# k-flouris/cmf

Measured on AMD Instinct MI355X. Metric: log-density evals/sec (JtJ-cholesky path), MNIST D=784 d=64 bs=512, higher is better.
Workload: dtype f32 (3x3 tangent convs as bf16x3 split MFMA, fp32 accumulate); 1 GPU; C3: MNIST-shaped (1,28,28) uint8-range + U[0,1) noise, non-square flow d=64, cholesky J^T J log-det + g_ij off-diagonal L1 + reconstruction, eval/no_grad; per_gpu_batch=512, global_batch=512, D=784, latent_dimension=64, parallelism=dp1

## Files before the change

cmf_amd/csrc/conv_block_head.hip:

```cpp
#include <stdint.h>

#include "common.h"

namespace {

typedef __bf16 bf16x8 __attribute__((ext_vector_type(8)));
typedef __bf16 bf16x2 __attribute__((ext_vector_type(2)));
typedef float f32x2 __attribute__((ext_vector_type(2)));
typedef unsigned u32x4 __attribute__((ext_vector_type(4)));

constexpr int HID = 64, KJ = HID * 9, NT = 512, ROWS = 16, ND = 25, HALO = 8, XB = 4;
constexpr int SLICE = HID * 16;
static_assert(2 * KJ > 2 * NT && 2 * KJ <= 3 * NT && (2 * KJ - 2 * NT) % 64 == 0, "phase B: two units per thread, a third for whole waves");
constexpr int W1_FRAGS = 9 * 4 * 2 * 2 * 64;

__device__ __forceinline__ unsigned pack_hi(float a, float b, float& ra, float& rb) {
  bf16x2 h = __builtin_convertvector(f32x2{a, b}, bf16x2);
  const unsigned bits = __builtin_bit_cast(unsigned, h);
  ra = a - __builtin_bit_cast(float, bits << 16);
  rb = b - __builtin_bit_cast(float, bits & 0xffff0000u);
  return bits;
}
__device__ __forceinline__ unsigned pack_lo(float a, float b) {
  bf16x2 h = __builtin_convertvector(f32x2{a, b}, bf16x2);
  return __builtin_bit_cast(unsigned, h);
}

__global__ void pack_block_weight_kernel(const float* __restrict__ w, u32x4* __restrict__ out) {
  const int idx = blockIdx.x * 256 + threadIdx.x;
  if (idx >= W1_FRAGS) return;
  const int l = idx & 63, hl = (idx >> 6) & 1, ks = (idx >> 7) & 1, ct = (idx >> 8) & 3, t1 = idx >> 10;
  const int c = 16 * ct + (l & 15), ci0 = 32 * ks + 8 * (l >> 4);
  unsigned r[4];
#pragma unroll
  for (int jj = 0; jj < 4; ++jj) {
    const float v0 = w[((ci0 + 2 * jj) * HID + c) * 9 + t1], v1 = w[((ci0 + 2 * jj + 1) * HID + c) * 9 + t1];
    float ra, rb;
    const unsigned h = pack_hi(v0, v1, ra, rb);
    r[jj] = hl ? pack_lo(ra, rb) : h;
  }
  out[idx] = u32x4{r[0], r[1], r[2], r[3]};
}

struct Tile {
  int row0, s0, xb, Ws, H, W, live;
  __device__ __forceinline__ bool slot(int p, int& row, int& col, int& po) const {
    const int s = s0 + (p & 1);
    row = row0 + (p >> 1);
    col = live ? 2 * s + ((row + live - 1) & 1) : s;
    po = row * Ws + s;
    return row < H && s < Ws;
  }
};

__device__ __forceinline__ void load_w1(u32x4 (&b)[2][2], const u32x4* __restrict__ wp, int ct, int lane, int t1) {
#pragma unroll
  for (int ks = 0; ks < 2; ++ks)
#pragma unroll
    for (int hl = 0; hl < 2; ++hl) b[ks][hl] = wp[(((t1 * 4 + ct) * 2 + ks) * 2 + hl) * 64 + lane];
}

template <int HALF, int CP>
__device__ __forceinline__ void build_half(const u32x4* __restrict__ wp, const u32x4* As, float* Ks, const float* Gs,
                                           const unsigned long long* ha, const int* ctr, int ct, int lane) {
  constexpr int D0 = HALF ? 12 : 0, NDH = HALF ? 13 : 12;
  const f32x4 zero = {0.f, 0.f, 0.f, 0.f};
  f32x4 acc[NDH];
  u32x4 af[9][2][2], bw[2][2][2];
#pragma unroll
  for (int i = 0; i < NDH; ++i) acc[i] = zero;
  load_w1(bw[0], wp, ct, lane, 0);
#pragma unroll
  for (int t2 = 0; t2 < 9; ++t2)
#pragma unroll
    for (int ks = 0; ks < 2; ++ks)
#pragma unroll
      for (int hl = 0; hl < 2; ++hl) af[t2][ks][hl] = As[((t2 * 2 + ks) * 2 + hl) * 64 + lane];
#pragma unroll
  for (int t1 = 0; t1 < 9; ++t1) {
    if (t1 < 8) load_w1(bw[(t1 + 1) & 1], wp, ct, lane, t1 + 1);
#pragma unroll
    for (int t2 = 0; t2 < 9; ++t2) {
      const int d = (t1 / 3 + t2 / 3) * 5 + t1 % 3 + t2 % 3;
      if (d >= D0 && d < D0 + NDH) {
#pragma unroll
        for (int ks = 0; ks < 2; ++ks) {
          const bf16x8 ah = __builtin_bit_cast(bf16x8, af[t2][ks][0]), al = __builtin_bit_cast(bf16x8, af[t2][ks][1]);
          const bf16x8 bh = __builtin_bit_cast(bf16x8, bw[t1 & 1][ks][0]), bl = __builtin_bit_cast(bf16x8, bw[t1 & 1][ks][1]);
          acc[d - D0] = __builtin_amdgcn_mfma_f32_16x16x32_bf16(al, bh, acc[d - D0], 0, 0, 0);
          acc[d - D0] = __builtin_amdgcn_mfma_f32_16x16x32_bf16(ah, bl, acc[d - D0], 0, 0, 0);
          acc[d - D0] = __builtin_amdgcn_mfma_f32_16x16x32_bf16(ah, bh, acc[d - D0], 0, 0, 0);
        }
      }
    }
  }
  const int c = 16 * ct + (lane & 15);
#pragma unroll
  for (int dl = 0; dl < NDH; ++dl) {
    const int d = D0 + dl;
#pragma unroll
    for (int i = 0; i < 4; ++i) {
      const int row = 4 * (lane >> 4) + i, p = row / CP, o = row % CP;
      const int at = ctr[p];
      const bool on = at >= 0 && ((ha[at + (d / 5 - 2) * HALO + d % 5 - 2] >> c) & 1);
      float v = on ? acc[dl][i] : 0.f;
      if (d == 12) v = Gs[c * ROWS + row] + v;
      Ks[((p * ND + d) * HID + c) * CP + o] = v;
    }
  }
}

template <int R, int CP>
__device__ __forceinline__ void phase_b(const float* __restrict__ w2, const float* Gs, const unsigned long long* um, u32x4* As, int tid) {
  int q[R], rh[R];
  float acc[R][8];
#pragma unroll
  for (int r = 0; r < R; ++r) {
    const int u = tid + r * NT;
    rh[r] = u >= KJ, q[r] = u - rh[r] * KJ;
#pragma unroll
    for (int i = 0; i < 8; ++i) acc[r][i] = 0.f;
  }
#pragma unroll 8
  for (int c = 0; c < HID; ++c) {
    float w[R];
#pragma unroll
    for (int r = 0; r < R; ++r) w[r] = w2[c * KJ + q[r]];
#pragma unroll
    for (int r = 0; r < R; ++r) {
      const f32x4 g0 = *reinterpret_cast<const f32x4*>(&Gs[c * ROWS + rh[r] * 8]), g1 = *reinterpret_cast<const f32x4*>(&Gs[c * ROWS + rh[r] * 8 + 4]);
#pragma unroll
      for (int k = 0; k < 4; ++k) {
        acc[r][k] = fmaf(g0[k], w[r], acc[r][k]);
        acc[r][4 + k] = fmaf(g1[k], w[r], acc[r][4 + k]);
      }
    }
  }
  unsigned short* A16 = reinterpret_cast<unsigned short*>(As);
#pragma unroll
  for (int r = 0; r < R; ++r) {
    const int ci = q[r] / 9, tap = q[r] - ci * 9, ks = ci >> 5, kq = (ci >> 3) & 3, j = ci & 7;
#pragma unroll
    for (int i = 0; i < 8; ++i) {
      const int row = rh[r] * 8 + i, p = row / CP;
      const float e = ((um[p * 9 + tap] >> ci) & 1) ? acc[r][i] : 0.f;
      float ra, rb;
      const unsigned h = pack_hi(e, 0.f, ra, rb);
      const unsigned l = pack_lo(ra, 0.f);
      const int at = ((tap * 2 + ks) * 2 * 64 + kq * 16 + row) * 8 + j;
      A16[at] = (unsigned short)(h & 0xffffu);
      A16[at + 64 * 8] = (unsigned short)(l & 0xffffu);
    }
  }
}

template <int CP>
__global__ __launch_bounds__(NT, 2) void conv_block_head_kernel(cmf_conv_tangent_args a, int tiles_x, int tiles_per_sample, int ntiles) {
  constexpr int P = ROWS / CP, TR = P / 2 > 0 ? P / 2 : 1, PU = P / 2;
  static_assert(P >= 2, "two output columns per tile");
  __shared__ __attribute__((aligned(16))) float Ks[ROWS * ND * HID];
  __shared__ __attribute__((aligned(16))) u32x4 As[9 * 2 * 2 * 64];
  __shared__ __attribute__((aligned(16))) float Gs[HID * ROWS];
  __shared__ unsigned long long um[P * 9];
  __shared__ unsigned long long ha[HALO * HALO];
  __shared__ unsigned long long hl[HALO * HALO];
  __shared__ unsigned long long alv[P];
  __shared__ int ctr[P];

  const int per = (ntiles + 7) >> 3;
  const int item = (int)(blockIdx.x & 7) * per + (int)(blockIdx.x >> 3);
  if (item >= ntiles) return;
  const int b = item / tiles_per_sample, tl = item - b * tiles_per_sample, ty = tl / tiles_x, tx = tl - ty * tiles_x;
  const int tid = threadIdx.x, lane = tid & 63, wv = __builtin_amdgcn_readfirstlane(tid >> 6);
  const int H = a.H, W = a.W, cout = a.head_cout;
  Tile T;
  T.H = H, T.W = W, T.live = a.live, T.Ws = a.live ? W >> 1 : W, T.row0 = ty * TR, T.s0 = 2 * tx, T.xb = a.live ? 4 * tx : 2 * tx;
  const int y0 = T.row0 - 2, x0 = T.xb - 2;

  if (tid < P * 9) {
    const int p = tid / 9, tap = tid - p * 9;
    int row, col, po;
    unsigned long long m = 0;
    if (T.slot(p, row, col, po)) {
      const int r = row + tap / 3 - 1, c = col + tap % 3 - 1;
      if (r >= 0 && r < H && c >= 0 && c < W)
        m = *reinterpret_cast<const unsigned long long*>(reinterpret_cast<const unsigned char*>(a.block_m1) + (long long)b * a.block_m1_np +
                                                         (long long)(r * W + c) * (HID / 8));
    }
    um[tid] = m;
  } else if (tid >= 256 && tid < 256 + HALO * HALO) {
    const int q = tid - 256, r = y0 + (q >> 3), c = x0 + (q & 7);
    unsigned long long m = 0;
    if (r >= 0 && r < H && c >= 0 && c < W)
      m = *reinterpret_cast<const unsigned long long*>(reinterpret_cast<const unsigned char*>(a.f) + (long long)b * a.f_np +
                                                       (long long)(r * W + c) * (HID / 8));
    ha[q] = m;
    hl[q] = m;
  }
  for (int p = wv; p < P; p += NT / 64) {
    int row, col, po;
    const bool ok = T.slot(p, row, col, po);
    bool on = false;
    if (ok) on = a.head_a[(long long)b * a.head_a_np + (long long)lane * a.head_a_c + (long long)(row * W + col) * a.head_a_px] > 0.f;
    const unsigned long long bal = __ballot(on);
    if (lane == 0) {
      alv[p] = bal;
      ctr[p] = ok ? (row - y0) * HALO + (col - x0) : -1;
    }
#pragma unroll
    for (int o = 0; o < CP; ++o) Gs[(lane * P + p) * CP + o] = (on && o < cout) ? a.head_w[o * HID + lane] : 0.f;
  }
  __syncthreads();
  if (tid < P) {
    int row, col, po;
    if (T.slot(tid, row, col, po)) hl[ctr[tid]] |= alv[tid];
  }

  if (wv < (2 * KJ - 2 * NT) / 64)
    phase_b<3, CP>(a.w, Gs, um, As, tid);
  else
    phase_b<2, CP>(a.w, Gs, um, As, tid);
  __syncthreads();

  {
    const u32x4* wp = reinterpret_cast<const u32x4*>(a.block_w1);
    if (wv < 4)
      build_half<0, CP>(wp, As, Ks, Gs, ha, ctr, wv & 3, lane);
    else
      build_half<1, CP>(wp, As, Ks, Gs, ha, ctr, wv & 3, lane);
  }
  __syncthreads();

  const int nsl = a.nc >> 4, cl = lane >> 2;
  const f32x4 zero = {0.f, 0.f, 0.f, 0.f};
  for (int unit = wv; unit < nsl * 2; unit += NT / 64) {
    const int sl = unit >> 1, ph = unit & 1;
    int prow[PU], pcol[PU], ppo[PU];
    bool pok[PU];
    int ylo = H, yhi = -1, xlo = W, xhi = -1;
#pragma unroll
    for (int k = 0; k < PU; ++k) {
      pok[k] = T.slot(ph * PU + k, prow[k], pcol[k], ppo[k]);
      if (pok[k]) {
        ylo = min(ylo, prow[k] - 2), yhi = max(yhi, prow[k] + 2);
        xlo = min(xlo, pcol[k] - 2), xhi = max(xhi, pcol[k] + 2);
      }
    }
    if (yhi < 0) continue;
    ylo = max(ylo, 0), yhi = min(yhi, H - 1), xlo = max(xlo, 0), xhi = min(xhi, W - 1);
    const float* hb = a.x + (long long)b * a.x_np + sl * SLICE + lane * 4;
    f32x4 acc[PU][CP];
#pragma unroll
    for (int k = 0; k < PU; ++k)
#pragma unroll
      for (int o = 0; o < CP; ++o) acc[k][o] = zero;

    for (int y = ylo; y <= yhi; ++y) {
#pragma unroll 1
      for (int xs = xlo; xs <= xhi; xs += XB) {
        f32x4 v[XB][4];
#pragma unroll
        for (int xi = 0; xi < XB; ++xi) {
#pragma unroll
          for (int ch = 0; ch < 4; ++ch) v[xi][ch] = zero;
          const int x = xs + xi;
          if (x <= xhi) {
            const unsigned long long m = hl[(y - y0) * HALO + (x - x0)];
            const float* src = hb + (long long)(y * W + x) * a.x_px;
#pragma unroll
            for (int ch = 0; ch < 4; ++ch)
              if ((m >> (ch * 16 + cl)) & 1) v[xi][ch] = *reinterpret_cast<const f32x4*>(src + ch * 256);
          }
        }
#pragma unroll
        for (int xi = 0; xi < XB; ++xi) {
          const int x = xs + xi;
#pragma unroll
          for (int k = 0; k < PU; ++k) {
            const int dy = y - prow[k] + 2, dx = x - pcol[k] + 2;
            if (x <= xhi && pok[k] && dy >= 0 && dy < 5 && dx >= 0 && dx < 5) {
              const float* coef = &Ks[(((ph * PU + k) * ND + dy * 5 + dx) * HID + cl) * CP];
#pragma unroll
              for (int ch = 0; ch < 4; ++ch) {
                const float* e4 = static_cast<const float*>(__builtin_assume_aligned(coef + ch * 16 * CP, CP < 4 ? 8 : 16));
#pragma unroll
                for (int o = 0; o < CP; ++o) {
                  const float e = e4[o];
#pragma unroll
                  for (int q = 0; q < 4; ++q) acc[k][o][q] = fmaf(e, v[xi][ch][q], acc[k][o][q]);
                }
              }
            }
          }
        }
      }
    }

    constexpr int N = 4 * CP;
#pragma unroll
    for (int k = 0; k < PU; ++k) {
      float val[N];
#pragma unroll
      for (int o = 0; o < CP; ++o)
#pragma unroll
        for (int q = 0; q < 4; ++q) val[4 * o + q] = acc[k][o][q];
#pragma unroll
      for (int s = 0; s < 4; ++s) {
        const int off = 32 >> s, n = N >> s;
        if (n >= 2) {
          const bool hi = lane & off;
#pragma unroll
          for (int i = 0; i < n / 2; ++i) {
            const float mine = hi ? val[n / 2 + i] : val[i], send = hi ? val[i] : val[n / 2 + i];
            val[i] = mine + __shfl_xor(send, off, 64);
          }
        } else {
          val[0] += __shfl_xor(val[0], off, 64);
        }
      }
      if (pok[k]) {
        float* yb = a.head_y + (long long)b * a.head_y_np + (long long)ppo[k] * a.head_y_px + sl * 16 + (lane & 3) * 4;
        constexpr int KEEP = N >= 16 ? N / 16 : 1;
#pragma unroll
        for (int i = 0; i < KEEP; ++i) {
          const int idx = ((cl * N) >> 4) + i, o = idx >> 2;
          if (o < cout && (N >= 16 || !(lane & 4))) yb[(long long)o * a.head_y_co + (idx & 3)] = val[i];
        }
      }
    }
  }
}

template <int CP>
int launch(const cmf_conv_tangent_args& a, hipStream_t s) {
  constexpr int P = ROWS / CP, TR = P / 2;
  const int Ws = a.live ? a.W / 2 : a.W;
  const long long tiles_x = (Ws + 1) / 2, tiles = tiles_x * ((a.H + TR - 1) / TR), ntiles = tiles * a.np;
  if (ntiles > 0x7ffffff0LL) return CMF_ERANGE;
  const int grid = 8 * (int)((ntiles + 7) / 8);
  hipLaunchKernelGGL(conv_block_head_kernel<CP>, dim3(grid), dim3(NT), 0, s, a, (int)tiles_x, (int)tiles, (int)ntiles);
  CMF_LAUNCH_CHECK();
  return 0;
}

}

extern "C" int cmf_pack_block_weight(const float* w, void* out, long long* out_bytes, void* stream) {
  if (!out) {
    if (!out_bytes) return CMF_EINVAL;
    *out_bytes = (long long)W1_FRAGS * 16;
    return 0;
  }
  if (!w || (uintptr_t)out % 16 || (uintptr_t)w % 4) return CMF_EINVAL;
  hipLaunchKernelGGL(pack_block_weight_kernel, dim3((W1_FRAGS + 255) / 256), dim3(256), 0, (hipStream_t)stream, w, (u32x4*)out);
  CMF_LAUNCH_CHECK();
  return 0;
}

int cmf_conv_block_head(const cmf_conv_tangent_args& a, hipStream_t s) {
  if (!a.x || !a.w || !a.f || !a.block_w1 || !a.block_m1 || !a.head_w || !a.head_a || !a.head_y) return CMF_EINVAL;
  if (a.r && a.r != a.x) return CMF_EINVAL;
  if (a.fmode != CMF_F_RELU_BITS || a.taps != 9 || a.cin != HID || a.cout != HID) return CMF_EINVAL;
  if (a.head_cout < 1 || a.head_cout > 8 || a.np <= 0 || a.H <= 0 || a.W <= 0 || a.nc <= 0 || a.nc % 16) return CMF_EINVAL;
  if (a.bias || a.fo || a.ymask || a.mask_out || a.seed || a.live < 0 || a.live > 2 || (a.live && a.W % 2)) return CMF_EINVAL;
  if (!((a.W % 14 == 0 && a.H % 2 == 0) || (a.W % 8 == 0 && a.H % 4 == 0))) return CMF_EINVAL;
  const long long HW = (long long)a.H * a.W;
  if (HW > (1 << 24)) return CMF_ERANGE;
  if (a.x_ci != 16 || a.x_sl != SLICE) return CMF_EINVAL;
  if ((a.x_np | a.x_px | a.head_y_np | a.head_y_co | a.head_y_px) % 4) return CMF_EINVAL;
  if (a.x_px < (long long)HID * a.nc || a.head_y_px < a.nc) return CMF_EINVAL;
  if ((uintptr_t)a.x % 16 || (uintptr_t)a.head_y % 16 || (uintptr_t)a.w % 4 || (uintptr_t)a.head_w % 4 || (uintptr_t)a.block_w1 % 16)
    return CMF_EINVAL;
  if ((uintptr_t)a.f % 8 || a.f_np % 8 || a.f_np < HW * (HID / 8)) return CMF_EINVAL;
  if ((uintptr_t)a.block_m1 % 8 || a.block_m1_np % 8 || a.block_m1_np < HW * (HID / 8)) return CMF_EINVAL;
  const int cp = a.head_cout <= 2 ? 2 : a.head_cout <= 4 ? 4 : 8;
  return cp == 2 ? launch<2>(a, s) : cp == 4 ? launch<4>(a, s) : launch<8>(a, s);
}
```

cmf_amd/csrc/probe_front.hip:

```cpp
#include <stdint.h>

#include "common.h"

namespace {

constexpr int HID = 64, NT = 256, SLICE = HID * 16;
constexpr int MAXT = 50;
constexpr int MAXCLS = 32;
constexpr int PASS = 64;

__global__ __launch_bounds__(NT) void probe_apply_kernel(cmf_probe_apply_args a, int nitems) {
  __shared__ __attribute__((aligned(16))) float Rs[MAXCLS * HID];
  __shared__ __attribute__((aligned(16))) float Ts[MAXT * PASS];
  __shared__ int tcls[MAXT], toff[MAXT];
  __shared__ int nterm;

  const int per = (nitems + 7) >> 3;
  const int item = (int)(blockIdx.x & 7) * per + (int)(blockIdx.x >> 3);
  if (item >= nitems) return;
  const int H = a.H, W = a.W, HW = H * W;
  const int b = item / HW, p = item - b * HW;
  const int tid = threadIdx.x, lane = tid & 63, wv = tid >> 6;
  const int ncls = a.ns * 16;
  const f32x4 zero = {0.f, 0.f, 0.f, 0.f};

  unsigned long long live = ~0ull;
  if (a.ymask)
    live = *reinterpret_cast<const unsigned long long*>(reinterpret_cast<const unsigned char*>(a.ymask) + (long long)b * a.ymask_np +
                                                        (long long)p * (HID / 8));

  if (wv == 0) {
    int cls = -1, off = 0;
    if (lane < 25 * a.cin) {
      const int w = lane / a.cin, c = lane - w * a.cin;
      const int r = p / W + w / 5 - 2, col = p % W + w % 5 - 2;
      if (r >= 0 && r < H && col >= 0 && col < W) {
        const int q = r * W + col, k = a.cls[c * HW + q];
        if (k >= 0 && k < ncls) {
          cls = k;
          off = (int)(c * a.t_c + q * a.t_px);
        }
      }
    }
    const unsigned long long bal = __ballot(cls >= 0);
    if (cls >= 0) {
      const int pos = __popcll(bal & ((1ull << lane) - 1ull));
      tcls[pos] = cls;
      toff[pos] = off;
    }
    if (lane == 0) nterm = __popcll(bal);
  }

  {
    const int co = tid >> 2, k4 = (tid & 3) * 4;
    const float* rb = a.r + (long long)b * a.r_np + (long long)p * a.r_px + tid * 4;
    for (int s = 0; s < a.ns; ++s) {
      f32x4 v = zero;
      if ((live >> co) & 1) v = *reinterpret_cast<const f32x4*>(rb + s * SLICE);
#pragma unroll
      for (int m = 0; m < 4; ++m) Rs[(s * 16 + k4 + m) * HID + (co & 15) * 4 + (co >> 4)] = v[m];
    }
  }
  __syncthreads();

  const int n = nterm, nsl = a.nc >> 4, cg = lane >> 2, quad = lane & 3;
  const float* tb = a.t + (long long)b * a.t_np;
  for (int s0 = 0; s0 < nsl; s0 += PASS / 16) {
    const int w4 = (nsl - s0 < PASS / 16 ? nsl - s0 : PASS / 16) * 4;
    if (s0) __syncthreads();
    for (int i = tid; i < n * w4; i += NT) {
      const int j = i / w4, x = i - j * w4;
      *reinterpret_cast<f32x4*>(&Ts[j * PASS + 4 * x]) = *reinterpret_cast<const f32x4*>(tb + toff[j] + s0 * 16 + 4 * x);
    }
    __syncthreads();
    const int sl = s0 + wv;
    if (sl >= nsl) continue;
    f32x4 acc[4] = {zero, zero, zero, zero};
    for (int j = 0; j < n; ++j) {
      const f32x4 c4 = *reinterpret_cast<const f32x4*>(&Rs[tcls[j] * HID + cg * 4]);
      const f32x4 t4 = *reinterpret_cast<const f32x4*>(&Ts[j * PASS + wv * 16 + quad * 4]);
#pragma unroll
      for (int i = 0; i < 4; ++i)
#pragma unroll
        for (int k = 0; k < 4; ++k) acc[i][k] = fmaf(c4[i], t4[k], acc[i][k]);
    }
    float* yb = a.y + (long long)b * a.y_np + (long long)p * a.y_px + sl * SLICE + quad * 4;
#pragma unroll
    for (int i = 0; i < 4; ++i) {
      const int co = cg + 16 * i;
      if ((live >> co) & 1) *reinterpret_cast<f32x4*>(yb + co * 16) = acc[i];
    }
  }
}

bool fits_i32(long long v) { return v >= 0 && v <= 0x7fffffffLL; }

}

extern "C" int cmf_probe_apply(const cmf_probe_apply_args* ap, void* stream) {
  if (!ap) return CMF_EINVAL;
  const cmf_probe_apply_args& a = *ap;
  if (!a.r || !a.t || !a.cls || !a.y) return CMF_EINVAL;
  if (a.np <= 0 || a.H <= 0 || a.W <= 0 || a.nc <= 0 || a.nc % 16) return CMF_EINVAL;
  if (a.cin < 1 || 25 * a.cin > MAXT || a.ns < 1 || a.ns * 16 > MAXCLS) return CMF_EINVAL;
  if ((a.r_np | a.r_px | a.t_np | a.t_c | a.t_px | a.y_np | a.y_px) % 4) return CMF_EINVAL;
  if ((uintptr_t)a.r % 16 || (uintptr_t)a.t % 16 || (uintptr_t)a.y % 16) return CMF_EINVAL;
  if (a.r_np < 0 || a.t_np < 0 || a.y_np < 0 || a.t_c < 0) return CMF_EINVAL;
  if (a.r_px < (long long)a.ns * SLICE || a.y_px < (long long)HID * a.nc || a.t_px < a.nc) return CMF_EINVAL;
  const long long HW = (long long)a.H * a.W;
  if (a.ymask && ((uintptr_t)a.ymask % 8 || a.ymask_np % 8 || a.ymask_np < HW * (HID / 8))) return CMF_EINVAL;
  if (HW > (1 << 24) || !fits_i32(a.cin * a.t_c + HW * a.t_px + a.nc)) return CMF_ERANGE;
  const long long nitems = HW * a.np;
  if (nitems > 0x7ffffff0LL) return CMF_ERANGE;
  const int grid = 8 * (int)((nitems + 7) / 8);
  hipLaunchKernelGGL(probe_apply_kernel, dim3(grid), dim3(NT), 0, (hipStream_t)stream, a, (int)nitems);
  CMF_LAUNCH_CHECK();
  return 0;
}
```

Measured before the change: 1564 evals/s.

## Use fp32 MFMA for phase B and software-pipeline halo loads with buffer loads

Phase B's per-thread scalar FMA outer product is replaced by 16x16x4 fp32 MFMA tiles, split across waves as five or four column tiles each. The halo gather in the tangent accumulation loop becomes a rolling pipeline of inline-asm buffer_load_dwordx4 over a full 8-wide row. Masked channels are dropped through an out-of-range offset, and explicit vmcnt waits let loads for the next row overlap compute on the current one. The aim is to cut phase B ALU time and hide global-load latency, at the cost of hand-managed waitcnt, more registers (a v[8][4] buffer) and fragile inline asm.

```diff
diff --git a/cmf_amd/csrc/conv_block_head.hip b/cmf_amd/csrc/conv_block_head.hip
--- a/cmf_amd/csrc/conv_block_head.hip
+++ b/cmf_amd/csrc/conv_block_head.hip
@@ -9,9 +9,9 @@
 typedef float f32x2 __attribute__((ext_vector_type(2)));
 typedef unsigned u32x4 __attribute__((ext_vector_type(4)));
 
-constexpr int HID = 64, KJ = HID * 9, NT = 512, ROWS = 16, ND = 25, HALO = 8, XB = 4;
+constexpr int HID = 64, KJ = HID * 9, NT = 512, ROWS = 16, ND = 25, HALO = 8;
 constexpr int SLICE = HID * 16;
-static_assert(2 * KJ > 2 * NT && 2 * KJ <= 3 * NT && (2 * KJ - 2 * NT) % 64 == 0, "phase B: two units per thread, a third for whole waves");
+static_assert(KJ == 16 * (4 * 5 + 4 * 4), "phase B: 36 column tiles of 16, five for waves 0 - 3 and four for waves 4 - 7");
 constexpr int W1_FRAGS = 9 * 4 * 2 * 2 * 64;
 
 __device__ __forceinline__ unsigned pack_hi(float a, float b, float& ra, float& rb) {
@@ -110,40 +110,33 @@
   }
 }
 
-template <int R, int CP>
-__device__ __forceinline__ void phase_b(const float* __restrict__ w2, const float* Gs, const unsigned long long* um, u32x4* As, int tid) {
-  int q[R], rh[R];
-  float acc[R][8];
-#pragma unroll
-  for (int r = 0; r < R; ++r) {
-    const int u = tid + r * NT;
-    rh[r] = u >= KJ, q[r] = u - rh[r] * KJ;
-#pragma unroll
-    for (int i = 0; i < 8; ++i) acc[r][i] = 0.f;
-  }
-#pragma unroll 8
-  for (int c = 0; c < HID; ++c) {
-    float w[R];
-#pragma unroll
-    for (int r = 0; r < R; ++r) w[r] = w2[c * KJ + q[r]];
-#pragma unroll
-    for (int r = 0; r < R; ++r) {
-      const f32x4 g0 = *reinterpret_cast<const f32x4*>(&Gs[c * ROWS + rh[r] * 8]), g1 = *reinterpret_cast<const f32x4*>(&Gs[c * ROWS + rh[r] * 8 + 4]);
-#pragma unroll
-      for (int k = 0; k < 4; ++k) {
-        acc[r][k] = fmaf(g0[k], w[r], acc[r][k]);
-        acc[r][4 + k] = fmaf(g1[k], w[r], acc[r][4 + k]);
-      }
-    }
+template <int NTL, int CP>
+__device__ __forceinline__ void phase_b(const float* __restrict__ w2, const float* Gs, const unsigned long long* um, u32x4* As, int t0, int lane) {
+  float g[HID / 4];
+#pragma unroll
+  for (int kk = 0; kk < HID / 4; ++kk) g[kk] = Gs[(4 * kk + (lane >> 4)) * ROWS + (lane & 15)];
+  const f32x4 zero = {0.f, 0.f, 0.f, 0.f};
+  f32x4 acc[NTL];
+#pragma unroll
+  for (int t = 0; t < NTL; ++t) acc[t] = zero;
+  const float* wl = w2 + (lane >> 4) * KJ + 16 * t0 + (lane & 15);
+#pragma unroll
+  for (int kk = 0; kk < HID / 4; ++kk) {
+    float w[NTL];
+#pragma unroll
+    for (int t = 0; t < NTL; ++t) w[t] = wl[4 * kk * KJ + 16 * t];
+#pragma unroll
+    for (int t = 0; t < NTL; ++t) acc[t] = __builtin_amdgcn_mfma_f32_16x16x4f32(g[kk], w[t], acc[t], 0, 0, 0);
   }
   unsigned short* A16 = reinterpret_cast<unsigned short*>(As);
 #pragma unroll
-  for (int r = 0; r < R; ++r) {
-    const int ci = q[r] / 9, tap = q[r] - ci * 9, ks = ci >> 5, kq = (ci >> 3) & 3, j = ci & 7;
-#pragma unroll
-    for (int i = 0; i < 8; ++i) {
-      const int row = rh[r] * 8 + i, p = row / CP;
-      const float e = ((um[p * 9 + tap] >> ci) & 1) ? acc[r][i] : 0.f;
+  for (int t = 0; t < NTL; ++t) {
+    const int q = 16 * (t0 + t) + (lane & 15);
+    const int ci = q / 9, tap = q - ci * 9, ks = ci >> 5, kq = (ci >> 3) & 3, j = ci & 7;
+#pragma unroll
+    for (int i = 0; i < 4; ++i) {
+      const int row = 4 * (lane >> 4) + i, p = row / CP;
+      const float e = ((um[p * 9 + tap] >> ci) & 1) ? acc[t][i] : 0.f;
       float ra, rb;
       const unsigned h = pack_hi(e, 0.f, ra, rb);
       const unsigned l = pack_lo(ra, 0.f);
@@ -151,6 +144,35 @@
       A16[at] = (unsigned short)(h & 0xffffu);
       A16[at + 64 * 8] = (unsigned short)(l & 0xffffu);
     }
+  }
+}
+
+typedef int i32x4 __attribute__((ext_vector_type(4)));
+constexpr int H_RECORDS = 0x7fffff00, H_DROP = 0x7ffffff0;
+__device__ __forceinline__ i32x4 halo_rsrc(const float* p) {
+  const unsigned long long u = reinterpret_cast<unsigned long long>(p);
+  i32x4 d;
+  d[0] = __builtin_amdgcn_readfirstlane((int)(unsigned)u);
+  d[1] = __builtin_amdgcn_readfirstlane((int)((unsigned)(u >> 32) & 0xffffu));
+  d[2] = H_RECORDS;
+  d[3] = 0x00020000;
+  return d;
+}
+template <int N>
+__device__ __forceinline__ void wait_halo(f32x4 (&v)[4]) {
+  asm volatile("s_waitcnt vmcnt(%4)" : "+v"(v[0]), "+v"(v[1]), "+v"(v[2]), "+v"(v[3]) : "n"(N));
+}
+__device__ __forceinline__ void wait_halo_n(f32x4 (&v)[4], int n) {
+  static_assert(HALO == 8, "cases below");
+  switch (n) {
+    case 0: wait_halo<0>(v); break;
+    case 1: wait_halo<4>(v); break;
+    case 2: wait_halo<8>(v); break;
+    case 3: wait_halo<12>(v); break;
+    case 4: wait_halo<16>(v); break;
+    case 5: wait_halo<20>(v); break;
+    case 6: wait_halo<24>(v); break;
+    default: wait_halo<28>(v); break;
   }
 }
 
@@ -216,10 +238,10 @@
     if (T.slot(tid, row, col, po)) hl[ctr[tid]] |= alv[tid];
   }
 
-  if (wv < (2 * KJ - 2 * NT) / 64)
-    phase_b<3, CP>(a.w, Gs, um, As, tid);
+  if (wv < 4)
+    phase_b<5, CP>(a.w, Gs, um, As, 5 * wv, lane);
   else
-    phase_b<2, CP>(a.w, Gs, um, As, tid);
+    phase_b<4, CP>(a.w, Gs, um, As, 20 + 4 * (wv - 4), lane);
   __syncthreads();
 
   {
@@ -248,52 +270,67 @@
     }
     if (yhi < 0) continue;
     ylo = max(ylo, 0), yhi = min(yhi, H - 1), xlo = max(xlo, 0), xhi = min(xhi, W - 1);
-    const float* hb = a.x + (long long)b * a.x_np + sl * SLICE + lane * 4;
+    const float* hb = a.x + (long long)b * a.x_np + sl * SLICE;
     f32x4 acc[PU][CP];
 #pragma unroll
     for (int k = 0; k < PU; ++k)
 #pragma unroll
       for (int o = 0; o < CP; ++o) acc[k][o] = zero;
 
-    for (int y = ylo; y <= yhi; ++y) {
-#pragma unroll 1
-      for (int xs = xlo; xs <= xhi; xs += XB) {
-        f32x4 v[XB][4];
-#pragma unroll
-        for (int xi = 0; xi < XB; ++xi) {
-#pragma unroll
-          for (int ch = 0; ch < 4; ++ch) v[xi][ch] = zero;
-          const int x = xs + xi;
-          if (x <= xhi) {
-            const unsigned long long m = hl[(y - y0) * HALO + (x - x0)];
-            const float* src = hb + (long long)(y * W + x) * a.x_px;
-#pragma unroll
-            for (int ch = 0; ch < 4; ++ch)
-              if ((m >> (ch * 16 + cl)) & 1) v[xi][ch] = *reinterpret_cast<const f32x4*>(src + ch * 256);
-          }
-        }
-#pragma unroll
-        for (int xi = 0; xi < XB; ++xi) {
-          const int x = xs + xi;
-#pragma unroll
-          for (int k = 0; k < PU; ++k) {
-            const int dy = y - prow[k] + 2, dx = x - pcol[k] + 2;
-            if (x <= xhi && pok[k] && dy >= 0 && dy < 5 && dx >= 0 && dx < 5) {
-              const float* coef = &Ks[(((ph * PU + k) * ND + dy * 5 + dx) * HID + cl) * CP];
-#pragma unroll
-              for (int ch = 0; ch < 4; ++ch) {
-                const float* e4 = static_cast<const float*>(__builtin_assume_aligned(coef + ch * 16 * CP, CP < 4 ? 8 : 16));
-#pragma unroll
-                for (int o = 0; o < CP; ++o) {
-                  const float e = e4[o];
-#pragma unroll
-                  for (int q = 0; q < 4; ++q) acc[k][o][q] = fmaf(e, v[xi][ch][q], acc[k][o][q]);
-                }
-              }
+    f32x4 v[HALO][4];
+    auto issue = [&](f32x4 (&r)[4], int y, int xi) {
+      const bool in = xlo + xi <= xhi;
+      const int x = in ? xlo + xi : xhi;
+      const unsigned long long m = in ? hl[(y - y0) * HALO + (x - x0)] : 0ull;
+      const i32x4 rs = halo_rsrc(hb + (long long)(y * W + x) * a.x_px);
+      int o[4];
+#pragma unroll
+      for (int ch = 0; ch < 4; ++ch) o[ch] = ((m >> (ch * 16 + cl)) & 1) ? lane * 16 : H_DROP;
+      asm volatile(
+          "s_nop 4\n\t"
+          "buffer_load_dwordx4 %0, %4, %8, 0 offen\n\t"
+          "buffer_load_dwordx4 %1, %5, %8, 0 offen offset:1024\n\t"
+          "buffer_load_dwordx4 %2, %6, %8, 0 offen offset:2048\n\t"
+          "buffer_load_dwordx4 %3, %7, %8, 0 offen offset:3072"
+          : "=&v"(r[0]), "=&v"(r[1]), "=&v"(r[2]), "=&v"(r[3])
+          : "v"(o[0]), "v"(o[1]), "v"(o[2]), "v"(o[3]), "s"(rs)
+          : "memory");
+    };
+    auto apply = [&](const f32x4 (&r)[4], int y, int xi) {
+      const int x = xlo + xi;
+#pragma unroll
+      for (int k = 0; k < PU; ++k) {
+        const int dy = y - prow[k] + 2, dx = x - pcol[k] + 2;
+        if (x <= xhi && pok[k] && dy >= 0 && dy < 5 && dx >= 0 && dx < 5) {
+          const float* coef = &Ks[(((ph * PU + k) * ND + dy * 5 + dx) * HID + cl) * CP];
+#pragma unroll
+          for (int ch = 0; ch < 4; ++ch) {
+            const float* e4 = static_cast<const float*>(__builtin_assume_aligned(coef + ch * 16 * CP, CP < 4 ? 8 : 16));
+#pragma unroll
+            for (int o = 0; o < CP; ++o) {
+              const float e = e4[o];
+#pragma unroll
+              for (int q = 0; q < 4; ++q) acc[k][o][q] = fmaf(e, r[ch][q], acc[k][o][q]);
             }
           }
         }
       }
+    };
+#pragma unroll
+    for (int xi = 0; xi < HALO; ++xi) issue(v[xi], ylo, xi);
+#pragma unroll 1
+    for (int y = ylo; y < yhi; ++y) {
+#pragma unroll
+      for (int xi = 0; xi < HALO; ++xi) {
+        wait_halo_n(v[xi], HALO - 1);
+        apply(v[xi], y, xi);
+        issue(v[xi], y + 1, xi);
+      }
+    }
+#pragma unroll
+    for (int xi = 0; xi < HALO; ++xi) {
+      wait_halo_n(v[xi], HALO - 1 - xi);
+      apply(v[xi], yhi, xi);
     }
 
     constexpr int N = 4 * CP;
```

Measured after the change: 1577 evals/s, median of 6. About the same (+0.8%).

## Rewrite probe apply as per-wave MFMA over pixel runs with software pipelining

Applied to the files above, without the earlier changes.

Replaces the one-block-per-pixel kernel, which staged R and T in shared memory and used scalar FMAs, with a kernel where each wave handles a run of consecutive pixels and computes the class-to-output contraction with 16x16x4 f32 MFMA. A per-wave class-to-offset table replaces the ballot-compacted term list, so zero-filled rows stand in for missing classes. Buffer loads with out-of-range offsets drop masked rows and stores. The next pixel's lookups and loads are prefetched while the current one computes. Adds template specialisations on ns and whether nc divides the pass width, plus compile-time knobs for run length and tiles per wave, at the cost of more register pressure and harder-to-check bounds logic.

```diff
diff --git a/cmf_amd/csrc/probe_front.hip b/cmf_amd/csrc/probe_front.hip
--- a/cmf_amd/csrc/probe_front.hip
+++ b/cmf_amd/csrc/probe_front.hip
@@ -4,92 +4,169 @@
 
 namespace {
 
-constexpr int HID = 64, NT = 256, SLICE = HID * 16;
+constexpr int HID = 64, NT = 256, NW = NT / 64, SLICE = HID * 16;
 constexpr int MAXT = 50;
 constexpr int MAXCLS = 32;
-constexpr int PASS = 64;
-
-__global__ __launch_bounds__(NT) void probe_apply_kernel(cmf_probe_apply_args a, int nitems) {
-  __shared__ __attribute__((aligned(16))) float Rs[MAXCLS * HID];
-  __shared__ __attribute__((aligned(16))) float Ts[MAXT * PASS];
-  __shared__ int tcls[MAXT], toff[MAXT];
-  __shared__ int nterm;
-
-  const int per = (nitems + 7) >> 3;
-  const int item = (int)(blockIdx.x & 7) * per + (int)(blockIdx.x >> 3);
-  if (item >= nitems) return;
-  const int H = a.H, W = a.W, HW = H * W;
-  const int b = item / HW, p = item - b * HW;
-  const int tid = threadIdx.x, lane = tid & 63, wv = tid >> 6;
-  const int ncls = a.ns * 16;
-  const f32x4 zero = {0.f, 0.f, 0.f, 0.f};
-
-  unsigned long long live = ~0ull;
-  if (a.ymask)
-    live = *reinterpret_cast<const unsigned long long*>(reinterpret_cast<const unsigned char*>(a.ymask) + (long long)b * a.ymask_np +
-                                                        (long long)p * (HID / 8));
-
-  if (wv == 0) {
-    int cls = -1, off = 0;
-    if (lane < 25 * a.cin) {
-      const int w = lane / a.cin, c = lane - w * a.cin;
-      const int r = p / W + w / 5 - 2, col = p % W + w % 5 - 2;
-      if (r >= 0 && r < H && col >= 0 && col < W) {
-        const int q = r * W + col, k = a.cls[c * HW + q];
-        if (k >= 0 && k < ncls) {
-          cls = k;
-          off = (int)(c * a.t_c + q * a.t_px);
-        }
+constexpr int PASS = 4;
+#ifndef CMF_PROBE_RUN
+#define CMF_PROBE_RUN 8
+#endif
+#ifndef CMF_PROBE_TPW
+#define CMF_PROBE_TPW 4
+#endif
+constexpr int RUN = CMF_PROBE_RUN;
+constexpr int TPW = CMF_PROBE_TPW;
+constexpr int DROP = 0x40000000;
+static_assert(TPW == 1 || TPW == 2 || TPW == 4, "tiles per wave");
+
+typedef unsigned u32x4 __attribute__((ext_vector_type(4)));
+typedef unsigned u32x2 __attribute__((ext_vector_type(2)));
+typedef int i32x4 __attribute__((ext_vector_type(4)));
+
+__device__ float zero_row[PASS * 16];
+
+template <int NS>
+struct Pixel {
+  int voff[TPW];
+  int o[4 * NS];
+};
+
+template <int NS, bool WHOLE>
+__global__ __launch_bounds__(NT) void probe_apply_kernel(cmf_probe_apply_args a, int nunits) {
+  __shared__ __attribute__((aligned(16))) int tab[NW][MAXCLS];
+
+  const int lane = threadIdx.x & 63, wv = __builtin_amdgcn_readfirstlane((int)threadIdx.x >> 6);
+  const int per = (int)gridDim.x >> 3;
+  const int unit = ((int)(blockIdx.x & 7) * per + (int)(blockIdx.x >> 3)) * NW + wv;
+  if (unit >= nunits) return;
+  constexpr int TG = 4 / TPW;
+  const int H = a.H, W = a.W, HW = H * W, nr = (HW + RUN - 1) / RUN;
+  const int t0 = (unit % TG) * TPW, run = unit / TG, b = run / nr, p0 = (run - b * nr) * RUN, p1 = p0 + RUN < HW ? p0 + RUN : HW;
+  const int i = lane & 15, g = lane >> 4, lane_off = i * 64 + g * 16;
+  const int nsl = a.nc >> 4, npass = (nsl + PASS - 1) / PASS;
+
+  const float* tb = a.t + (long long)b * a.t_np;
+  const float* rb = a.r + (long long)b * a.r_np;
+  float* yb = a.y + (long long)b * a.y_np;
+  const unsigned char* ym = a.ymask ? reinterpret_cast<const unsigned char*>(a.ymask) + (long long)b * a.ymask_np : nullptr;
+  int* tw = tab[wv];
+
+  const bool wl = lane < 25 * a.cin;
+  const int wpos = lane / a.cin, wc = lane - wpos * a.cin, dy = wpos / 5 - 2, dx = wpos % 5 - 2;
+
+  const auto dcls = __builtin_amdgcn_make_buffer_rsrc(const_cast<signed char*>(a.cls), 0, a.cin * HW, 0x00020000);
+  const auto dym = __builtin_amdgcn_make_buffer_rsrc(const_cast<unsigned char*>(ym), 0, ym ? HW * (HID / 8) : 0, 0x00020000);
+
+  auto look = [&](int p, int r, int col, int& k, int& off, u32x2& live) {
+    const int rr = r + dy, cc = col + dx, q = rr * W + cc;
+    const bool in = (int)wl & (int)(p < p1) & (int)(rr >= 0) & (int)(rr < H) & (int)(cc >= 0) & (int)(cc < W);
+    k = (signed char)__builtin_amdgcn_raw_buffer_load_b8(dcls, in ? wc * HW + q : DROP, 0, 0);
+    live = __builtin_amdgcn_raw_buffer_load_b64(dym, p < p1 ? p * (HID / 8) : DROP, 0, 0);
+    __builtin_amdgcn_sched_barrier(0);
+    off = in ? (int)(wc * a.t_c + q * a.t_px) : -1;
+  };
+  auto build = [&](int p, int k, int off, u32x2 lv, Pixel<NS>& s) {
+    if (lane < 16 * NS) tw[lane] = -1;
+    __builtin_amdgcn_wave_barrier();
+    if (off >= 0 && k >= 0 && k < 16 * NS) tw[k] = off;
+    __builtin_amdgcn_wave_barrier();
+#pragma unroll
+    for (int rs = 0; rs < NS; ++rs) {
+      const i32x4 v = *reinterpret_cast<const i32x4*>(&tw[16 * rs + 4 * g]);
+#pragma unroll
+      for (int m = 0; m < 4; ++m) s.o[4 * rs + m] = v[m];
+    }
+    __builtin_amdgcn_wave_barrier();
+    unsigned long long live = (unsigned long long)lv[1] << 32 | lv[0];
+    if (!ym) live = p < p1 ? ~0ull : 0;
+#pragma unroll
+    for (int t = 0; t < TPW; ++t) s.voff[t] = (live >> (16 * (t0 + t) + i)) & 1 ? lane_off + 1024 * (t0 + t) : DROP;
+  };
+  auto load_r = [&](int p, const Pixel<NS>& s, u32x4 (&R)[NS][TPW]) {
+    const auto d = __builtin_amdgcn_make_buffer_rsrc(const_cast<float*>(rb + (long long)p * a.r_px), 0, NS * SLICE * 4, 0x00020000);
+#pragma unroll
+    for (int rs = 0; rs < NS; ++rs)
+#pragma unroll
+      for (int t = 0; t < TPW; ++t) R[rs][t] = __builtin_amdgcn_raw_buffer_load_b128(d, s.voff[t] + rs * SLICE * 4, 0, 0);
+  };
+  auto load_a = [&](const Pixel<NS>& s, int ps, float (&A)[4 * NS][PASS]) {
+#pragma unroll
+    for (int m = 0; m < 4 * NS; ++m) {
+      const float* row = s.o[m] >= 0 ? tb + s.o[m] + ps * PASS * 16 + i : zero_row + i;
+#pragma unroll
+      for (int j = 0; j < PASS; ++j) {
+        int cj = j;
+        if constexpr (!WHOLE) cj = ps * PASS + j < nsl ? j : nsl - 1 - ps * PASS;
+        A[m][j] = row[cj * 16];
       }
     }
-    const unsigned long long bal = __ballot(cls >= 0);
-    if (cls >= 0) {
-      const int pos = __popcll(bal & ((1ull << lane) - 1ull));
-      tcls[pos] = cls;
-      toff[pos] = off;
-    }
-    if (lane == 0) nterm = __popcll(bal);
-  }
-
-  {
-    const int co = tid >> 2, k4 = (tid & 3) * 4;
-    const float* rb = a.r + (long long)b * a.r_np + (long long)p * a.r_px + tid * 4;
-    for (int s = 0; s < a.ns; ++s) {
-      f32x4 v = zero;
-      if ((live >> co) & 1) v = *reinterpret_cast<const f32x4*>(rb + s * SLICE);
-#pragma unroll
-      for (int m = 0; m < 4; ++m) Rs[(s * 16 + k4 + m) * HID + (co & 15) * 4 + (co >> 4)] = v[m];
-    }
-  }
-  __syncthreads();
-
-  const int n = nterm, nsl = a.nc >> 4, cg = lane >> 2, quad = lane & 3;
-  const float* tb = a.t + (long long)b * a.t_np;
-  for (int s0 = 0; s0 < nsl; s0 += PASS / 16) {
-    const int w4 = (nsl - s0 < PASS / 16 ? nsl - s0 : PASS / 16) * 4;
-    if (s0) __syncthreads();
-    for (int i = tid; i < n * w4; i += NT) {
-      const int j = i / w4, x = i - j * w4;
-      *reinterpret_cast<f32x4*>(&Ts[j * PASS + 4 * x]) = *reinterpret_cast<const f32x4*>(tb + toff[j] + s0 * 16 + 4 * x);
-    }
-    __syncthreads();
-    const int sl = s0 + wv;
-    if (sl >= nsl) continue;
-    f32x4 acc[4] = {zero, zero, zero, zero};
-    for (int j = 0; j < n; ++j) {
-      const f32x4 c4 = *reinterpret_cast<const f32x4*>(&Rs[tcls[j] * HID + cg * 4]);
-      const f32x4 t4 = *reinterpret_cast<const f32x4*>(&Ts[j * PASS + wv * 16 + quad * 4]);
-#pragma unroll
-      for (int i = 0; i < 4; ++i)
-#pragma unroll
-        for (int k = 0; k < 4; ++k) acc[i][k] = fmaf(c4[i], t4[k], acc[i][k]);
-    }
-    float* yb = a.y + (long long)b * a.y_np + (long long)p * a.y_px + sl * SLICE + quad * 4;
-#pragma unroll
-    for (int i = 0; i < 4; ++i) {
-      const int co = cg + 16 * i;
-      if ((live >> co) & 1) *reinterpret_cast<f32x4*>(yb + co * 16) = acc[i];
-    }
+  };
+
+  int r2 = p0 / W, c2 = p0 - r2 * W;
+  auto step = [&]() {
+    if (++c2 == W) c2 = 0, ++r2;
+  };
+  int k0, off0, k1, off1;
+  u32x2 live0, live1;
+  Pixel<NS> cur, nxt;
+  u32x4 R[NS][TPW], Rn[NS][TPW];
+  float A[4 * NS][PASS], An[4 * NS][PASS];
+  look(p0, r2, c2, k0, off0, live0);
+  step();
+  look(p0 + 1, r2, c2, k1, off1, live1);
+  step();
+  build(p0, k0, off0, live0, cur);
+  load_r(p0, cur, R);
+  load_a(cur, 0, A);
+  __builtin_amdgcn_s_waitcnt(0x0f70);
+
+  for (int p = p0; p < p1; ++p) {
+    build(p + 1, k1, off1, live1, nxt);
+    look(p + 2, r2, c2, k1, off1, live1);
+    step();
+    load_r(p + 1, nxt, Rn);
+    float Rs[NS][TPW][4];
+#pragma unroll
+    for (int rs = 0; rs < NS; ++rs)
+#pragma unroll
+      for (int t = 0; t < TPW; ++t) {
+        const f32x4 rf = __builtin_bit_cast(f32x4, R[rs][t]);
+#pragma unroll
+        for (int s = 0; s < 4; ++s) Rs[rs][t][s] = cur.o[4 * rs + s] >= 0 ? rf[s] : 0.f;
+      }
+    float* yp = yb + (long long)p * a.y_px;
+    int ps = 0;
+    do {
+      if (ps + 1 < npass)
+        load_a(cur, ps + 1, An);
+      else
+        load_a(nxt, 0, An);
+#pragma unroll
+      for (int j = 0; j < PASS; ++j) {
+        const int sl = ps * PASS + j;
+        f32x4 acc[TPW];
+#pragma unroll
+        for (int t = 0; t < TPW; ++t) acc[t] = f32x4{0.f, 0.f, 0.f, 0.f};
+#pragma unroll
+        for (int m = 0; m < 4 * NS; ++m)
+#pragma unroll
+          for (int t = 0; t < TPW; ++t) acc[t] = __builtin_amdgcn_mfma_f32_16x16x4f32(A[m][j], Rs[m >> 2][t][m & 3], acc[t], 0, 0, 0);
+        const auto d = __builtin_amdgcn_make_buffer_rsrc(yp + (long long)sl * SLICE, 0, sl < nsl ? SLICE * 4 : 0, 0x00020000);
+#pragma unroll
+        for (int t = 0; t < TPW; ++t)
+          __builtin_amdgcn_raw_buffer_store_b128(__builtin_bit_cast(u32x4, acc[t]), d, cur.voff[t], 0, 0);
+        __builtin_amdgcn_sched_barrier(0);
+      }
+#pragma unroll
+      for (int m = 0; m < 4 * NS; ++m)
+#pragma unroll
+        for (int j = 0; j < PASS; ++j) A[m][j] = An[m][j];
+    } while (++ps < npass);
+#pragma unroll
+    for (int rs = 0; rs < NS; ++rs)
+#pragma unroll
+      for (int t = 0; t < TPW; ++t) R[rs][t] = Rn[rs][t];
+    cur = nxt;
   }
 }
 
@@ -112,8 +189,13 @@
   if (HW > (1 << 24) || !fits_i32(a.cin * a.t_c + HW * a.t_px + a.nc)) return CMF_ERANGE;
   const long long nitems = HW * a.np;
   if (nitems > 0x7ffffff0LL) return CMF_ERANGE;
-  const int grid = 8 * (int)((nitems + 7) / 8);
-  hipLaunchKernelGGL(probe_apply_kernel, dim3(grid), dim3(NT), 0, (hipStream_t)stream, a, (int)nitems);
+  const long long nunits = (HW + RUN - 1) / RUN * a.np * (4 / TPW);
+  if (nunits > 0x7ffffff0LL) return CMF_ERANGE;
+  const int grid = 8 * (int)((nunits + 8 * NW - 1) / (8 * NW));
+  const bool whole = a.nc % (16 * PASS) == 0;
+  auto* kernel = a.ns == 1 ? (whole ? probe_apply_kernel<1, true> : probe_apply_kernel<1, false>)
+                           : (whole ? probe_apply_kernel<2, true> : probe_apply_kernel<2, false>);
+  hipLaunchKernelGGL(kernel, dim3(grid), dim3(NT), 0, (hipStream_t)stream, a, (int)nunits);
   CMF_LAUNCH_CHECK();
   return 0;
 }
```

Result: no change. 1562 evals/s before, 1568 evals/s after, median of 6 (+0.4%).
